# wwood/smafa

Hardware: AMD Instinct MI355X
Metric: query seqs/sec (DB residues/sec in `residues_per_s`) vs roofline, 10M x 60aa DB, d<=5 (higher is better)
Workload: dtype u32

## Files before the change

smafa_amd/csrc/engine.hip:

```cpp
#include <hipcub/hipcub.hpp>
#include <cmath>

#include <algorithm>
#include <atomic>
#include <cstdarg>
#include <cstdio>
#include <cstdlib>
#include <cstring>
#include <string>
#include <vector>

#include "engine.h"
#include "scan_plan.h"
#include "host/packed.h"
#include "kernels.hip.h"
#include "index.hip.h"
#include "join.hip.h"
#include "components.hip.h"
#include "levels.hip.h"
#include "density.hip.h"
#include "peaks.hip.h"
#include "neighbours.hip.h"

namespace smafa {
// ... 640 lines not shown
        x.probe_block[j] = j <= thr0 ? probe_block[j] : 0;
        x.probe_cols[j] = (uint32_t)ix.col_begin[x.probe_block[j]] | ((uint32_t)ix.col_begin[x.probe_block[j] + 1] << 16);
    }
    ScanArgs a{};
    a.n_subjects = (uint32_t)db->n;
    a.hits = d_rows;
    a.cap = rows_cap;
    a.count = d_count;
    a.order = db->d_order;
    int cur_dev = -1;
    if (hipGetDevice(&cur_dev) == hipSuccess) {
        db->launch_device = cur_dev;
        if (cur_dev != db->device) db->launches_off_device++;
    }
    const uint32_t *qrec = qs->qrec.as<uint32_t>();
    const uint32_t per_launch = (uint32_t)((1ull << 31) / kIndexGroup / x.n_probes);
    for (uint32_t qb = q_begin; qb < q_end;) {
        const uint32_t qe = q_end - qb > per_launch ? qb + per_launch : q_end;
        x.q_begin = qb;
        x.q_end = qe;
        const uint64_t groups = (uint64_t)(qe - qb) * x.n_probes;
        const uint64_t grid = (groups * kIndexGroup + kIndexWg - 1u) / kIndexWg;
        const bool launched = for_shape(db->shape(), [&](auto ps, auto pq, auto w) {
            constexpr int PS = decltype(ps)::value, PQ = decltype(pq)::value, W = decltype(w)::value;
            hipLaunchKernelGGL((index_probe_kernel<PS, PQ, W>), dim3((uint32_t)grid), dim3(kIndexWg), 0, db->stream, db->d_planes, qrec, x, a);
            note_kernel(db, "smafa::index_probe_kernel<%d, %d, %d>", PS, PQ, W);
            return true;
        });
        if (!launched) return set_error(SMAFA_ERR_INVALID, "no index probe for %u/%u planes x %u words", db->P, db->PQ, db->W);
        HIP_TRY(hipGetLastError());
        db->last_launches++;
        qb = qe;
    }
    db->plan_lazy = 0;
    db->plan_tiles = 0;
    db->plan_qblocks = 1;
    db->index_probes++;
    return SMAFA_OK;
}

static int launch_tiles(smafa_db *db, smafa_qset *qs, uint32_t q_begin, uint32_t q_end, uint32_t tile_begin,
                        uint32_t tile_end, uint32_t k_tight, uint32_t thr0, smafa_hit *d_rows, uint64_t rows_cap,
                        unsigned long long *publish, bool per_query_bounds = false, unsigned long long *own_counter = nullptr) {
    ScanArgs a;
    const uint32_t nq = q_end - q_begin, n_tiles = tile_end - tile_begin;
    const bool per_query = k_tight || per_query_bounds;
    const ScanPlan plan = plan_scan(db->shape(), db->knobs, {thr0, nq, d_rows == nullptr && k_tight == 1, d_rows != nullptr, per_query, {db->zone_hist}});
    const uint32_t T = plan.T;
    a.tile_begin = tile_begin;
    a.tile_end = tile_end;
    a.n_wg_tiles = (n_tiles + plan.wg_waves * T - 1) / (plan.wg_waves * T);
    a.n_subjects = (uint32_t)db->n;
    a.q_begin = q_begin;
    a.q_end = q_end;
    a.qb_size = query_block_size(db->qb_override, (uint32_t)db->n_cu, (n_tiles + kWgWaves * T - 1) / (kWgWaves * T), nq,
                                 plan.whole_chunks ? (uint32_t)kChunk : 1u);
    a.thr = per_query ? qs->thr.as<uint32_t>() : nullptr;
    a.thr0 = thr0;
    a.cnt = qs->cnt.as<uint32_t>();
    a.cnt_stride = db->L + 1;
    a.k_tight = k_tight;
    a.use_filter = db->knobs.use_filter ? 1u : 0u;
    a.hits = d_rows;
    a.cap = rows_cap;
    a.count = db->ctrs.as<unsigned long long>();
    a.done = publish ? reinterpret_cast<uint32_t *>(db->ctrs.as<uint8_t>() + 256) : nullptr;
    a.publish = publish;
    if (own_counter) {
        a.count = own_counter;
        a.done = nullptr;
        a.publish = nullptr;
    }
    a.order = db->d_order;
    a.zone = db->d_zone;
    a.zone_on = plan.zone_on ? 1u : 0u;
    {
        const uint32_t n1 = db->L > 32u ? std::min(db->L - 32u, 32u) : 0u, kb = (uint32_t)SMAFA_ZONE_KEY_BITS;
        const uint32_t xw = n1 >= 2u * kb ? kb : n1 / 2u;
        a.key_xmask = xw ? (uint32_t)((1ull << xw) - 1ull) : 0u;
        a.key_zlo = xw;
        a.key_gate = db->zone_key_gate >= 0                  ? (uint32_t)db->zone_key_gate
                     : db->alphabet == SMAFA_ALPHABET_AA ? (uint32_t)SMAFA_ZONE_KEY_GATE
                                                         : (uint32_t)SMAFA_ZONE_KEY_GATE_NT;
    }
    const uint64_t n_qblocks = (q_end - q_begin + a.qb_size - 1) / a.qb_size;
    const uint64_t range_bytes = (uint64_t)n_tiles * (plan.reported_lazy ? db->W : db->P * db->W) * 1024u;
    a.stream_once = (db->stream_nt && (n_qblocks == 1 || range_bytes >= (256ull << 20))) ? 1u : 0u;
    const uint64_t grid = n_qblocks * a.n_wg_tiles;
    if (grid > 0x7fffffffull)
        return set_error(SMAFA_ERR_INVALID, "scan grid too large (%llu workgroups)", (unsigned long long)grid);
    int cur_dev = -1;
    if (hipGetDevice(&cur_dev) == hipSuccess) {
        db->launch_device = cur_dev;
        if (cur_dev != db->device) db->launches_off_device++;
    }
    const std::string id = scan_kernel_name(plan, db->shape());
    note_kernel(db, "%s", id.c_str());
    if (plan.zone_on) note_kernel(db, "%s (zone level on)", id.c_str());
    if (!launch_scan(db, qs->qrec.as<uint32_t>(), a, (uint32_t)grid, plan)) return set_error(SMAFA_ERR_INVALID, "no kernel %s", id.c_str());
    db->plan_lazy = plan.reported_lazy ? 1u : 0u;
    db->plan_tiles = T;
    db->plan_qblocks = (uint32_t)n_qblocks;
    HIP_TRY(hipGetLastError());
    db->last_launches++;
    return SMAFA_OK;
}

static int scan_range(smafa_db *db, smafa_qset *qs, uint32_t q_begin, uint32_t q_end, uint32_t max_div,
                      uint32_t k_tight, smafa_hit *d_hits, uint64_t cap, unsigned long long *d_count, uint32_t tile_begin = 0) {
    const uint32_t nq = q_end - q_begin;
    db->last_launches = 0;
    db->timed = false;
    db->call_timed = false;
    if (nq == 0 || db->n == 0) {
        HIP_TRY(hipMemsetAsync(d_count, 0, sizeof(unsigned long long), db->stream));
        return SMAFA_OK;
    }
    int prc = maybe_resort(db);
    if (prc) return prc;
    unsigned long long *d_ctr = db->ctrs.as<unsigned long long>();
    const uint32_t thr0 = std::min<uint32_t>(max_div, db->L);
    const uint32_t n_tiles = (uint32_t)((db->n + kWaveTile - 1) / kWaveTile);
    if (k_tight == 0) {
        if (db->index_mode >= 2 && db->knobs.use_filter && nq > 64u && db->W <= (uint32_t)kIndexMaxWords && thr0 + 1u <= std::min<uint32_t>(kIndexMaxBlocks, db->L) &&
            db->n >= db->index_min_rows && db->n < (1ull << 31) && (!index_current(db) || db->index.B < thr0 + 1u)) {
            bool build = db->index_mode == 2;
            if (!build) {
                if (db->index_debt_generation != db->generation) db->index_debt_ms = 0.0, db->index_debt_generation = db->generation;
                db->index_debt_ms += (double)nq * (double)db->n * (double)(db->P * db->W) * 1.7e-12;
                build = db->index_debt_ms >= 0.3 + (double)(thr0 + 1u) * (double)db->n * 1.0e-7;
            }
            if (build && db->index_failed_generation != db->generation + 1u) {
                if (index_build(db, thr0 + 1u) != SMAFA_OK) {
                    log_line(1, "block index not built (%s): scanning as before", smafa_last_error());
                    index_drop(db);
                    db->index_failed_generation = db->generation + 1u;
                }
            }
        }
        uint8_t probe_block[kIndexMaxBlocks];
        if (index_plan(db, thr0, nq, probe_block)) {
            hipLaunchKernelGGL(fill_u32_kernel, dim3(1), dim3(64), 0, db->stream, (uint32_t *)d_count, 0u, (uint64_t)2);
            HIP_TRY(hipEventRecord(db->ev0, db->stream));
            int rc = index_probe(db, qs, q_begin, q_end, thr0, probe_block, d_hits, cap, d_count);
            if (rc) return rc;
            HIP_TRY(hipEventRecord(db->ev1, db->stream));
            db->timed = true;
            return SMAFA_OK;
        }
        const bool own = nq <= 64u;
        if (own) hipLaunchKernelGGL(fill_u32_kernel, dim3(1), dim3(64), 0, db->stream, (uint32_t *)d_count, 0u, (uint64_t)2);
        HIP_TRY(hipEventRecord(db->ev0, db->stream));
        int rc = launch_tiles(db, qs, q_begin, q_end, tile_begin, n_tiles, 0, thr0, d_hits, cap, own ? nullptr : d_count, false,
                              own ? d_count : nullptr);
        if (rc) return rc;
        HIP_TRY(hipEventRecord(db->ev1, db->stream));
        db->timed = true;
        return SMAFA_OK;
    }
    const bool count_first = k_tight >= db->count_first_k && !prefilter_prunes(db->shape(), db->knobs, thr0);
    const uint32_t sample_tiles = (count_first && db->kth_sample_div && n_tiles >= db->kth_sample_min_tiles &&
                                   n_tiles / db->kth_sample_div >= 1u &&
                                   (uint64_t)k_tight * 4u <= (uint64_t)(n_tiles / db->kth_sample_div) * kWaveTile)
                                      ? n_tiles / db->kth_sample_div : 0u;
    uint64_t scratch_rows = 0;
    if (!count_first || sample_tiles) {
// ... 1480 lines not shown
```

smafa_amd/csrc/kernels.hip.h:

```cpp
#pragma once

#include <type_traits>
#include <hip/hip_runtime.h>
#include <stdint.h>

#include "../../include/smafa_amd.h"
#include "scan_plan.h"

namespace smafa {

constexpr int kStageRows = 256;
__host__ __device__ constexpr int scan_min_waves(int ps, int w, int t) {
    const int regs = t * ps * w * 4 + 40;
    return regs <= 64 ? 8 : regs <= 80 ? 6 : regs <= 96 ? 5 : regs <= 128 ? 4 : regs <= 168 ? 3 : 2;
}
#ifndef SMAFA_CASCADE
#define SMAFA_CASCADE 1
#endif
#ifndef SMAFA_WIDE_AND_PAIR
#define SMAFA_WIDE_AND_PAIR 1
#endif
#ifndef SMAFA_SIGN_COMPARE
#define SMAFA_SIGN_COMPARE 1
#endif
// ... 680 lines not shown
                    }
                }
            }
        }
        if (more) commit(buf ^ 1, qc + kChunk);
        __syncthreads();
        if (!SEED && a.hits) flush_rows(a, rs, buf);
    }
    if (!SEED) finish_rows(a);
}

__device__ __forceinline__ void emit_direct(const ScanArgs &a, uint32_t q, uint32_t pos, uint32_t dist) {
    smafa_hit h;
    h.query = q;
    h.subject = a.order[pos];
    h.dist = dist;
    const unsigned long long together = __ballot(1);
    const int first = __builtin_ctzll(together);
    unsigned long long g = 0;
    if ((int)__lane_id() == first) g = atomicAdd(a.count, (unsigned long long)__builtin_popcountll(together));
    g = shfl_u64(g, first) + lanes_below(together);
    if (g < a.cap) a.hits[g] = h;
}

constexpr int kZoneTiles = SMAFA_ZONE_TILES;

#ifndef SMAFA_ZONE_WAVES_10
#define SMAFA_ZONE_WAVES_10 5
#endif
#ifndef SMAFA_ZONE_SGPR_ZONE
#define SMAFA_ZONE_SGPR_ZONE 1
#endif
#ifndef SMAFA_ZONE_VGPR_MASK
#define SMAFA_ZONE_VGPR_MASK 6
#endif
#ifndef SMAFA_ZONE_OPAQUE_BUF
#define SMAFA_ZONE_OPAQUE_BUF 1
#endif
#ifndef SMAFA_ZONE_FULL_DMA
#define SMAFA_ZONE_FULL_DMA 1
#endif
#ifndef SMAFA_ZONE_NLIVE
#define SMAFA_ZONE_NLIVE 1
#endif
#ifndef SMAFA_ZONE_WAVES_4
#define SMAFA_ZONE_WAVES_4 6
#endif
#ifndef SMAFA_ZONE_WAVES_6
#define SMAFA_ZONE_WAVES_6 6
#endif
#ifndef SMAFA_ZONE_WAVES_DIRECT_AA
#define SMAFA_ZONE_WAVES_DIRECT_AA 7
#endif
#ifndef SMAFA_ZONE_KEYS
#define SMAFA_ZONE_KEYS 3
#endif
#ifndef SMAFA_ZONE_KEY_BITS
#define SMAFA_ZONE_KEY_BITS 12
#endif
#ifndef SMAFA_ZONE_KEY_GATE
#define SMAFA_ZONE_KEY_GATE 3
#endif
#ifndef SMAFA_ZONE_KEY_GATE_NT
#define SMAFA_ZONE_KEY_GATE_NT 2
#endif
#ifndef SMAFA_ZONE_KEY_HOIST
#define SMAFA_ZONE_KEY_HOIST 1
#endif
#ifndef SMAFA_ZONE_L2_LANES
#define SMAFA_ZONE_L2_LANES 1
#endif
#ifndef SMAFA_ZONE_F1_HOME_AA
#define SMAFA_ZONE_F1_HOME_AA 1
#endif
#ifndef SMAFA_ZONE_F1_HOME_NT
#define SMAFA_ZONE_F1_HOME_NT 0
#endif
__host__ __device__ constexpr int zone_f1_home(int ps, int w, bool direct) {
    return !(SMAFA_ZONE_L2_LANES && direct && w == 2 && SMAFA_ZONE_KEYS > 0) ? 0 : ps == 5 ? SMAFA_ZONE_F1_HOME_AA : SMAFA_ZONE_F1_HOME_NT;
}
#ifndef SMAFA_ZONE_KEY_BATCH
#define SMAFA_ZONE_KEY_BATCH 1
#endif
__host__ __device__ constexpr int zone_key_sets(int w, bool direct) { return direct && w == 2 ? SMAFA_ZONE_KEYS : 0; }
static_assert(SMAFA_ZONE_KEYS == 0 || SMAFA_ZONE_KEYS == 2 || SMAFA_ZONE_KEYS == 3, "SMAFA_ZONE_KEYS: 0, 2 or 3");
static_assert(SMAFA_ZONE_KEY_BITS >= 8 && SMAFA_ZONE_KEY_BITS <= 16, "SMAFA_ZONE_KEY_BITS: 8..16");

__host__ __device__ constexpr int zone_min_waves(int ps, int w, bool direct = false) {
    return (direct && ps == 5 && w == 2 && SMAFA_ZONE_TILES == 4) ? SMAFA_ZONE_WAVES_DIRECT_AA
           : ps * w <= 4 ? SMAFA_ZONE_WAVES_4 : (ps == 3 && w == 2) ? SMAFA_ZONE_WAVES_6 : ps * w <= 10 ? SMAFA_ZONE_WAVES_10 : 4;
}

template <int PS, int PQ, int W, bool FIXED, bool DIRECT = false>
__global__ __launch_bounds__(kZoneWgWaves * 64, zone_min_waves(PS, W, DIRECT)) void scan_zone_kernel(const uint4 *__restrict__ planes,
                                                           const uint32_t *__restrict__ qrec, ScanArgs a) {
    static_assert(FIXED || !DIRECT, "per-query bounds keep the staged form");
    constexpr int T = zone_tiles(PS, W, DIRECT);
    constexpr int RS = qrec_stride(PQ, W);
    constexpr int RV = RS / 4;
    constexpr int WGW = kZoneWgWaves;
    constexpr int NT = WGW * 64;
    constexpr int NV = (kChunk * RV + NT - 1) / NT;
    constexpr int FP = filter_plane(PQ);
    constexpr int BS = bound_slot(W);
    constexpr bool kPair = SMAFA_AND_PAIR && W > 1;
    __shared__ uint4 stage[2][kChunk * RV];
    __shared__ uint32_t nu_lds[2][kChunk];
    __shared__ RowStageT<(WGW == 1 ? 64 : kStageRows)> rs;
    constexpr int NS = zone_key_sets(W, DIRECT);
    constexpr int KB = SMAFA_ZONE_KEY_BITS;
    constexpr int KW = (1 << KB) / 32;
    __shared__ uint4 keymap[NS ? WGW * T * NS * KW / 4 : 1];
    constexpr int kF1Home = NS > 0 ? zone_f1_home(PS, W, DIRECT) : 0;
    constexpr bool kL2Lanes = NS > 0 && W == 2 && SMAFA_ZONE_L2_LANES;
    __shared__ uint4 f1_lds[kF1Home == 1 ? WGW * T * 64 : 1];
    int buf = 0;

    const uint32_t tid = threadIdx.x;
    const uint32_t lane = tid & 63u;
    const uint32_t wave = tid >> 6;
    if ((!DIRECT || NS == 0) && tid == 0) rs.n[0] = rs.n[1] = 0;
    const uint32_t wg_tile = blockIdx.x % a.n_wg_tiles;
    const uint32_t qblock = blockIdx.x / a.n_wg_tiles;
    const uint32_t tile0 = (uint32_t)__builtin_amdgcn_readfirstlane((int)(a.tile_begin + (wg_tile * WGW + wave) * T));
    const bool active = tile0 < a.tile_end;
    const uint32_t n_live = active ? min((uint32_t)T, a.tile_end - tile0) : 0u;
    const uint32_t q0 = a.q_begin + qblock * a.qb_size;
    const uint32_t q1 = min(q0 + a.qb_size, a.q_end);

    uint4 f0[T];
    uint4 f1_reg[kF1Home == 2 ? T : 1];
    auto load_filter = [&]() {
#pragma unroll
        for (int t = 0; t < T; t++) {
            const bool live = SMAFA_ZONE_NLIVE ? (uint32_t)t < n_live : tile0 + t < a.tile_end;
            f0[t] = planes[(size_t)(live ? tile0 + t : a.tile_begin) * (PS * W * 64) + (FP * W) * 64 + lane];
            if constexpr (kF1Home == 2) f1_reg[t] = planes[(size_t)(live ? tile0 + t : a.tile_begin) * (PS * W * 64) + (FP * W + 1) * 64 + lane];
        }
    };
    load_filter();
    uint4 vz = make_uint4(0u, 0u, 0u, 0u);
    if (lane < (uint32_t)T && tile0 + lane < a.tile_end) vz = a.zone[tile0 + lane];
    uint32_t zc0[T], zm0[T];
#pragma unroll
    for (int t = 0; t < T; t++) {
        zc0[t] = (uint32_t)__builtin_amdgcn_readlane((int)vz.x, t);
        zm0[t] = (uint32_t)__builtin_amdgcn_readlane((int)vz.y, t);
    }
    constexpr bool kMaskInVgpr = PS * W <= SMAFA_ZONE_VGPR_MASK;
    uint32_t zmv[T];
#pragma unroll
    for (int t = 0; t < T; t++) {
        zmv[t] = zm0[t];
        if (kMaskInVgpr) asm volatile("v_mov_b32 %0, %1" : "=v"(zmv[t]) : "s"(zm0[t]));
    }
    const bool zone_w1 = W > 1 && __ballot(vz.w != 0u) != 0ull;
    uint32_t zc1s[T], zm1s[T];
#pragma unroll
    for (int t = 0; t < T; t++) {
        zc1s[t] = NS > 0 ? (uint32_t)__builtin_amdgcn_readlane((int)vz.z, t) : 0u;
        zm1s[t] = NS > 0 ? (uint32_t)__builtin_amdgcn_readlane((int)vz.w, t) : 0u;
    }

    auto key_y = [&](uint32_t w0) -> uint32_t { return w0 >> (32 - KB); };
    auto key_x = [&](uint32_t w1) -> uint32_t { return w1 & a.key_xmask; };
    auto key_z = [&](uint32_t w1) -> uint32_t { return __builtin_amdgcn_ubfe(w1, a.key_zlo, KB); };
    constexpr bool kHoist = NS > 0 && SMAFA_ZONE_KEY_HOIST;
    bool key_hoist = false;
    if constexpr (kHoist) {
        uint32_t shared_keys = 0;
#pragma unroll
        for (int t = 0; t < T; t++) shared_keys |= key_y(zm0[t]) | key_x(zm1s[t]) | (NS > 2 ? key_z(zm1s[t]) : 0u);
        key_hoist = shared_keys == 0u;
    }
    uint32_t *const km = reinterpret_cast<uint32_t *>(keymap) + (size_t)__builtin_amdgcn_readfirstlane((int)wave) * (T * NS * KW);
    uint4 *const f1_home = f1_lds + (kF1Home == 1 ? (size_t)__builtin_amdgcn_readfirstlane((int)wave) * (T * 64) : 0);
    if constexpr (NS > 0) {
        uint4 *const km4 = reinterpret_cast<uint4 *>(km);
#pragma unroll
        for (int i = 0; i < T * NS * KW / 4; i += 64)
            if (i + 64 <= T * NS * KW / 4 || i + (int)lane < T * NS * KW / 4) km4[i + lane] = make_uint4(0u, 0u, 0u, 0u);
        __builtin_amdgcn_wave_barrier();
        asm volatile("s_waitcnt lgkmcnt(0)" ::: "memory");
#pragma unroll
        for (int t = 0; t < T; t++) {
            const bool live = (uint32_t)t < n_live;
            uint4 f1;
            if constexpr (kF1Home == 2) f1 = f1_reg[t];
            else f1 = planes[(size_t)(live ? tile0 + t : a.tile_begin) * (PS * W * 64) + (FP * W + 1) * 64 + lane];
            if constexpr (kF1Home == 1) f1_home[t * 64 + lane] = f1;
            const uint32_t w0[4] = {f0[t].x, f0[t].y, f0[t].z, f0[t].w};
            const uint32_t w1[4] = {f1.x, f1.y, f1.z, f1.w};
#pragma unroll
            for (int k = 0; k < 4; k++) {
                const uint32_t ky = key_y(w0[k]), kx = key_x(w1[k]);
                atomicOr(&km[(t * NS + 0) * KW + (ky >> 5)], 1u << (ky & 31u));
                atomicOr(&km[(t * NS + 1) * KW + (kx >> 5)], 1u << (kx & 31u));
                if (NS > 2) {
                    const uint32_t kz = key_z(w1[k]);
                    atomicOr(&km[(t * NS + (NS > 2 ? 2 : 0)) * KW + (kz >> 5)], 1u << (kz & 31u));
                }
            }
        }
        __builtin_amdgcn_wave_barrier();
        asm volatile("s_waitcnt lgkmcnt(0)" ::: "memory");
    }

    auto dma = [&](int b, uint32_t qc) {
        const uint32_t nqc = SMAFA_ZONE_FULL_DMA ? (uint32_t)kChunk : min((uint32_t)kChunk, q1 - qc);
        const uint4 *src = reinterpret_cast<const uint4 *>(qrec + (size_t)qc * RS);
#pragma unroll
        for (int v = 0; v < NV; v++) {
            const uint32_t idx = tid + v * NT;
            if (idx < nqc * RV)
                __builtin_amdgcn_global_load_lds((const __attribute__((address_space(1))) void *)(src + idx),
                                                 (__attribute__((address_space(3))) void *)(&stage[b][wave * 64 + v * NT]), 16, 0, 0);
        }
    };
    const uint32_t nu0 = ~a.thr0;
    auto load_bound = [&](uint32_t qc) -> uint32_t {
        return tid < min((uint32_t)kChunk, q1 - qc) ? ~ld_relaxed(a.thr + qc + tid) : 0u;
    };
    uint32_t nu_next = 0;
    auto read_record = [&](const uint4 *rec, uint32_t(&qw)[RS]) {
#pragma unroll
        for (int v = 0; v < RV; v++) {
            const uint4 x = rec[v];
            qw[4 * v + 0] = x.x;
            qw[4 * v + 1] = x.y;
            qw[4 * v + 2] = x.z;
            qw[4 * v + 3] = x.w;
        }
    };
    auto stream_compare = [&](uint32_t tile, const uint32_t(&qw)[RS], uint32_t q, int parity) {
        const uint32_t U = ~qw[BS];
        const uint4 *src = planes + (size_t)tile * (PS * W * 64) + lane;
        uint32_t d[4] = {0u, 0u, 0u, 0u};
#pragma unroll
        for (int w = 0; w < W; w++) {
            uint32_t extra = 0;
#pragma unroll
            for (int p = PS; p < PQ; p++) extra |= qw[qslot(PQ, W, p, w)];
            uint32_t m0 = extra, m1 = extra, m2 = extra, m3 = extra;
#pragma unroll
            for (int p = 0; p < PS; p++) {
                const uint4 v = src[(p * W + w) * 64];
                const uint32_t qv = qw[qslot(PQ, W, p, w)];
                m0 = or_xor(m0, v.x, qv);
                m1 = or_xor(m1, v.y, qv);
                m2 = or_xor(m2, v.z, qv);
                m3 = or_xor(m3, v.w, qv);
            }
            d[0] += __builtin_popcount(m0);
            d[1] += __builtin_popcount(m1);
            d[2] += __builtin_popcount(m2);
            d[3] += __builtin_popcount(m3);
        }
        const uint32_t subj0 = tile * kWaveTile + lane * 4u;
#pragma unroll
        for (int k = 0; k < 4; k++)
            if (d[k] <= U && subj0 + k < a.n_subjects) {
                if (DIRECT) emit_direct(a, q, subj0 + k, d[k]);
                else emit(a, rs, parity, q, subj0 + k, d[k]);
            }
    };
    auto load_head = [&](uint32_t qc) -> uint2 {
        return *reinterpret_cast<const uint2 *>(qrec + (size_t)(qc + lane) * RS);
    };
    uint2 head_next = make_uint2(0u, 0u);

    if (!DIRECT) {
        if (q0 < q1) {
            dma(0, q0);
            if (!FIXED && tid < (uint32_t)kChunk) nu_lds[0][tid] = load_bound(q0);
        }
        asm volatile("s_waitcnt vmcnt(0)" ::: "memory");
        __syncthreads();
    } else if (q0 < q1) {
        head_next = load_head(q0);
    }
    bool filter_on = a.use_filter != 0;
    uint32_t chunk_no = 0;
    for (uint32_t qc = q0; qc < q1; qc += kChunk, buf ^= 1, chunk_no++) {
        const uint32_t nqc = min((uint32_t)kChunk, q1 - qc);
        const bool more = qc + kChunk < q1;
        const uint2 head_cur = head_next;
        if (more) {
            if (DIRECT) {
                head_next = load_head(qc + kChunk);
            } else {
                dma(buf ^ 1, qc + kChunk);
                if (!FIXED) nu_next = load_bound(qc + kChunk);
            }
        }
        if (active) {
            const bool probe = a.use_filter && (filter_on || (chunk_no & 15u) == 0);
            if (probe) {
                uint32_t passes = 0;
                uint4 head = make_uint4(0u, 0u, 0u, 0u);
                if (DIRECT) head.x = head_cur.x, head.y = head_cur.y;
                else if (lane < nqc) head = stage[buf][lane * RV];
                const uint32_t hq0 = head.x, hq1 = W > 1 ? head.y : 0u;
                const uint32_t hnu = lane < nqc ? (FIXED ? nu0 : nu_lds[buf][lane]) : 0u;
                uint32_t nl = n_live;
                asm volatile("" : "+s"(nl));
                if (!SMAFA_ZONE_SGPR_ZONE) asm volatile("" : "+v"(vz.x), "+v"(vz.y));
                auto zone_keys = [&](auto slot) -> unsigned long long {
                    constexpr uint32_t t = decltype(slot)::value;
                    const uint32_t zc = SMAFA_ZONE_SGPR_ZONE ? zc0[t] : (uint32_t)__builtin_amdgcn_readlane((int)vz.x, (int)t);
                    const uint32_t zm = SMAFA_ZONE_SGPR_ZONE ? zm0[t] : (uint32_t)__builtin_amdgcn_readlane((int)vz.y, (int)t);
                    const uint32_t d0 = (hq0 ^ zc) & (kMaskInVgpr ? zmv[t] : zm);
                    uint32_t u = __builtin_popcount(d0) + hnu;
                    uint32_t d1 = 0;
                    if (zone_w1) {
                        const uint32_t zc1 = NS > 0 ? zc1s[t] : (uint32_t)__builtin_amdgcn_readlane((int)vz.z, (int)t);
                        const uint32_t zm1 = NS > 0 ? zm1s[t] : (uint32_t)__builtin_amdgcn_readlane((int)vz.w, (int)t);
                        d1 = (hq1 ^ zc1) & zm1;
                        u += __builtin_popcount(d1);
                    }
                    unsigned long long m = __ballot((int32_t)u < 0);
                    if constexpr (NS > 0) {
                        if ((uint32_t)__builtin_popcountll(m) >= a.key_gate) {
                            bool pass = false;
                            if ((int32_t)u < 0) {
                                const uint32_t s0 = hq0 ^ d0, s1 = hq1 ^ d1;
                                const uint32_t ky = key_y(s0), kx = key_x(s1);
                                const uint32_t vy = km[(t * NS + 0) * KW + (ky >> 5)];
                                const uint32_t vx = km[(t * NS + 1) * KW + (kx >> 5)];
                                uint32_t found = ((vy >> (ky & 31u)) & 1u) + ((vx >> (kx & 31u)) & 1u);
                                if (NS > 2) {
                                    const uint32_t kz = key_z(s1);
                                    const uint32_t vz_ = km[(t * NS + (NS > 2 ? 2 : 0)) * KW + (kz >> 5)];
                                    found += (vz_ >> (kz & 31u)) & 1u;
                                }
                                pass = found + ~u >= (uint32_t)NS;
                            }
                            m = __ballot(pass);
                        }
                    }
                    return m;
                };
                auto survivors = [&](auto slot, unsigned long long m) {
                    constexpr uint32_t t = decltype(slot)::value;
                    const uint32_t tile = tile0 + t;
                    const uint4 ft = f0[t];
                    while (m != 0ull) {
                        const int i = __builtin_ctzll(m);
                        asm("s_bitset0_b64 %0, %1" : "+s"(m) : "s"(i));
                        const uint32_t q0w = (uint32_t)__builtin_amdgcn_readlane((int)hq0, i);
                        const uint32_t nu = FIXED ? nu0 : (uint32_t)__builtin_amdgcn_readlane((int)hnu, i);
                        const uint32_t u0 = __builtin_popcount(ft.x ^ q0w) + nu;
                        const uint32_t u1 = __builtin_popcount(ft.y ^ q0w) + nu;
                        const uint32_t u2 = __builtin_popcount(ft.z ^ q0w) + nu;
                        const uint32_t u3 = __builtin_popcount(ft.w ^ q0w) + nu;
                        if (__ballot((int32_t)(or3(u0, u1, u2) | u3) < 0) == 0ull) continue;
                        uint32_t tile_r = tile;
                        asm volatile("" : "+s"(tile_r));
#if SMAFA_ZONE_OPAQUE_BUF
                        int buf_r = __builtin_amdgcn_readfirstlane(buf);
                        asm volatile("" : "+s"(buf_r));
#define SMAFA_ZONE_BUF buf_r
#else
#define SMAFA_ZONE_BUF buf
#endif
                        uint32_t qw[RS];
                        if constexpr (kL2Lanes) {
                            const uint32_t q1w = (uint32_t)__builtin_amdgcn_readlane((int)hq1, i);
                            uint4 v;
                            if constexpr (kF1Home == 1) v = f1_home[t * 64 + lane];
                            else if constexpr (kF1Home == 2) v = f1_reg[t];
                            else v = planes[(size_t)tile_r * (PS * W * 64) + (FP * W + 1) * 64 + lane];
                            const uint32_t m0 = or_xor(ft.x ^ q0w, v.x, q1w), m1 = or_xor(ft.y ^ q0w, v.y, q1w);
                            const uint32_t m2 = or_xor(ft.z ^ q0w, v.z, q1w), m3 = or_xor(ft.w ^ q0w, v.w, q1w);
                            if (kPair) {
                                const uint32_t sign = (__builtin_popcount(m0 & m1) + nu) | (__builtin_popcount(m2 & m3) + nu);
                                if (__ballot((int32_t)sign < 0) == 0ull) continue;
                            }
                            const uint32_t each = or3(__builtin_popcount(m0) + nu, __builtin_popcount(m1) + nu,
                                                      __builtin_popcount(m2) + nu) |
                                                  (__builtin_popcount(m3) + nu);
                            if (__ballot((int32_t)each < 0) == 0ull) continue;
                            read_record(reinterpret_cast<const uint4 *>(qrec + (size_t)(qc + (uint32_t)i) * RS), qw);
                            qw[BS] = nu;
                            passes++;
                            stream_compare(tile_r, qw, qc + (uint32_t)i, SMAFA_ZONE_BUF);
                            continue;
                        }
                        if (DIRECT) read_record(reinterpret_cast<const uint4 *>(qrec + (size_t)(qc + (uint32_t)i) * RS), qw);
                        else read_record(&stage[SMAFA_ZONE_BUF][(uint32_t)i * RV], qw);
                        qw[BS] = nu;
                        uint32_t m0 = ft.x ^ qw[0], m1 = ft.y ^ qw[0], m2 = ft.z ^ qw[0], m3 = ft.w ^ qw[0];
                        if (W > 1) {
                            const uint4 *src = planes + (size_t)tile_r * (PS * W * 64) + (FP * W) * 64 + lane;
#pragma unroll
                            for (int w = 1; w < W; w++) {
                                const uint4 v = src[w * 64];
                                m0 = or_xor(m0, v.x, qw[qslot(PQ, W, FP, w)]);
                                m1 = or_xor(m1, v.y, qw[qslot(PQ, W, FP, w)]);
                                m2 = or_xor(m2, v.z, qw[qslot(PQ, W, FP, w)]);
                                m3 = or_xor(m3, v.w, qw[qslot(PQ, W, FP, w)]);
                            }
                            if (kPair) {
                                const uint32_t sign = (__builtin_popcount(m0 & m1) + nu) | (__builtin_popcount(m2 & m3) + nu);
                                if (__ballot((int32_t)sign < 0) == 0ull) continue;
                            }
                            const uint32_t each = or3(__builtin_popcount(m0) + nu, __builtin_popcount(m1) + nu,
                                                      __builtin_popcount(m2) + nu) |
                                                  (__builtin_popcount(m3) + nu);
                            if (__ballot((int32_t)each < 0) == 0ull) continue;
                        }
                        passes++;
                        stream_compare(tile_r, qw, qc + (uint32_t)i, SMAFA_ZONE_BUF);
#undef SMAFA_ZONE_BUF
                    }
                };
                static_assert(T <= 8, "tile slots are spelled out below");
                auto each_slot = [&](auto &&f) {
                    f(std::integral_constant<uint32_t, 0>{});
                    if constexpr (T > 1) f(std::integral_constant<uint32_t, 1>{});
                    if constexpr (T > 2) f(std::integral_constant<uint32_t, 2>{});
                    if constexpr (T > 3) f(std::integral_constant<uint32_t, 3>{});
                    if constexpr (T > 4) f(std::integral_constant<uint32_t, 4>{});
                    if constexpr (T > 5) f(std::integral_constant<uint32_t, 5>{});
                    if constexpr (T > 6) f(std::integral_constant<uint32_t, 6>{});
                    if constexpr (T > 7) f(std::integral_constant<uint32_t, 7>{});
                };
                static_assert(!kHoist || (SMAFA_ZONE_NLIVE && SMAFA_ZONE_SGPR_ZONE),
                              "the two-phase form of the key-test kernels is written for SMAFA_ZONE_NLIVE = SMAFA_ZONE_SGPR_ZONE = 1");
                if constexpr (kHoist) {
                    unsigned long long ms[T];
                    if (key_hoist) {
                        const uint32_t ky = key_y(hq0), kx = key_x(hq1), kz = NS > 2 ? key_z(hq1) : 0u;
                        typedef const __attribute__((address_space(3))) uint32_t *lds_u32;
                        const uint32_t km_lds = (uint32_t)(uintptr_t)(__attribute__((address_space(3))) void *)km;
                        auto word_of = [&](uint32_t key) -> uint32_t {
                            uint32_t at;
                            asm("v_lshl_add_u32 %0, %1, 2, %2" : "=v"(at) : "v"(key >> 5), "s"(km_lds));
                            return at;
                        };
                        const uint32_t ay = word_of(ky), ax = word_of(kx), az = NS > 2 ? word_of(kz) : 0u;
                        const unsigned long long in_block = ~0ull >> (64u - nqc);
                        auto hoisted = [&](auto with_w1) {
                            if constexpr (SMAFA_ZONE_KEY_BATCH) {
                                uint32_t u[T];
                                bool test = false;
                                each_slot([&](auto slot) {
                                    constexpr uint32_t t = decltype(slot)::value;
                                    u[t] = __builtin_popcount((hq0 ^ zc0[t]) & (kMaskInVgpr ? zmv[t] : zm0[t])) + nu0;
                                    if (decltype(with_w1)::value) u[t] += __builtin_popcount((hq1 ^ zc1s[t]) & zm1s[t]);
                                    const unsigned long long m = __builtin_amdgcn_ballot_w64((int32_t)u[t] < 0) & in_block;
                                    ms[t] = t == 0u || nl > t ? m : 0ull;
                                    test = test || (uint32_t)__builtin_popcountll(ms[t]) >= a.key_gate;
                                });
                                if (test) {
                                    uint32_t g[T][3];
                                    each_slot([&](auto slot) {
                                        constexpr uint32_t t = decltype(slot)::value;
                                        g[t][0] = g[t][1] = g[t][2] = 0u;
                                        if ((int32_t)u[t] < 0) {
                                            g[t][0] = *(lds_u32)(uintptr_t)(ay + ((t * NS + 0) * KW) * 4u);
                                            g[t][1] = *(lds_u32)(uintptr_t)(ax + ((t * NS + 1) * KW) * 4u);
                                            if (NS > 2) g[t][2] = *(lds_u32)(uintptr_t)(az + ((t * NS + (NS > 2 ? 2 : 0)) * KW) * 4u);
                                        }
                                    });
                                    each_slot([&](auto slot) {
                                        constexpr uint32_t t = decltype(slot)::value;
                                        uint32_t found = __builtin_amdgcn_ubfe(g[t][0], ky, 1) + __builtin_amdgcn_ubfe(g[t][1], kx, 1);
                                        if (NS > 2) found += __builtin_amdgcn_ubfe(g[t][2], kz, 1);
                                        ms[t] &= __builtin_amdgcn_ballot_w64((int32_t)(u[t] - found) < -(int32_t)NS);
                                    });
                                }
                            } else {
                            auto one = [&](auto slot) -> unsigned long long {
                                constexpr uint32_t t = decltype(slot)::value;
                                uint32_t u = __builtin_popcount((hq0 ^ zc0[t]) & (kMaskInVgpr ? zmv[t] : zm0[t])) + nu0;
                                if (decltype(with_w1)::value) u += __builtin_popcount((hq1 ^ zc1s[t]) & zm1s[t]);
                                unsigned long long m = __builtin_amdgcn_ballot_w64((int32_t)u < 0) & in_block;
                                if ((uint32_t)__builtin_popcountll(m) >= a.key_gate) {
                                    if ((int32_t)u < 0) {
                                        uint32_t found = __builtin_amdgcn_ubfe(*(lds_u32)(uintptr_t)(ay + ((t * NS + 0) * KW) * 4u), ky, 1) +
                                                         __builtin_amdgcn_ubfe(*(lds_u32)(uintptr_t)(ax + ((t * NS + 1) * KW) * 4u), kx, 1);
                                        if (NS > 2) found += __builtin_amdgcn_ubfe(*(lds_u32)(uintptr_t)(az + ((t * NS + (NS > 2 ? 2 : 0)) * KW) * 4u), kz, 1);
                                        u -= found;
                                    }
                                    asm("" : "+v"(u));
                                    m &= __builtin_amdgcn_ballot_w64((int32_t)u < -(int32_t)NS);
                                }
                                return m;
                            };
                            each_slot([&](auto slot) {
                                constexpr uint32_t t = decltype(slot)::value;
                                ms[t] = t == 0u || nl > t ? one(slot) : 0ull;
                            });
                            }
                        };
                        if (zone_w1) hoisted(std::true_type{});
                        else hoisted(std::false_type{});
                    } else {
                        each_slot([&](auto slot) {
                            constexpr uint32_t t = decltype(slot)::value;
                            ms[t] = t == 0u || nl > t ? zone_keys(slot) : 0ull;
                        });
                    }
                    each_slot([&](auto slot) { survivors(slot, ms[decltype(slot)::value]); });
                } else {
                    each_slot([&](auto slot) {
                        constexpr uint32_t t = decltype(slot)::value;
                        if (SMAFA_ZONE_NLIVE ? nl > t : tile0 + t < a.tile_end) survivors(slot, zone_keys(slot));
                    });
                }
                filter_on = passes * 5u <= nqc * 8u;
            } else {
                for (uint32_t t = 0; t < (uint32_t)T; t++) {
                    const uint32_t tile = tile0 + t;
                    if (SMAFA_ZONE_NLIVE ? t >= n_live : tile >= a.tile_end) break;
                    uint4 s[PS * W];
                    uint32_t tile_d = tile;
                    asm volatile("" : "+s"(tile_d));
                    const uint4 *src = planes + (size_t)(SMAFA_ZONE_NLIVE ? tile_d : tile) * (PS * W * 64) + lane;
#pragma unroll
                    for (int i = 0; i < PS * W; i++) s[i] = src[i * 64];
                    const uint4 *rec = DIRECT ? reinterpret_cast<const uint4 *>(qrec + (size_t)qc * RS) : &stage[buf][0];
                    for (uint32_t i = 0; i < nqc; i++, rec += RV) {
                        uint32_t qw[RS];
                        read_record(rec, qw);
                        const uint32_t U = FIXED ? a.thr0 : ~nu_lds[buf][i];
                        uint32_t d[4];
#pragma unroll
                        for (int w = 0; w < W; w++) {
                            uint32_t extra = 0;
#pragma unroll
                            for (int p = PS; p < PQ; p++) extra |= qw[qslot(PQ, W, p, w)];
                            uint32_t m0 = extra, m1 = extra, m2 = extra, m3 = extra;
#pragma unroll
                            for (int p = 0; p < PS; p++) {
                                const uint4 v = s[p * W + w];
                                const uint32_t qv = qw[qslot(PQ, W, p, w)];
                                m0 = or_xor(m0, v.x, qv);
                                m1 = or_xor(m1, v.y, qv);
                                m2 = or_xor(m2, v.z, qv);
                                m3 = or_xor(m3, v.w, qv);
                            }
                            d[0] = (w ? d[0] : 0u) + __builtin_popcount(m0);
                            d[1] = (w ? d[1] : 0u) + __builtin_popcount(m1);
                            d[2] = (w ? d[2] : 0u) + __builtin_popcount(m2);
                            d[3] = (w ? d[3] : 0u) + __builtin_popcount(m3);
                        }
                        const uint32_t subj0 = tile * kWaveTile + lane * 4u;
#pragma unroll
                        for (int k = 0; k < 4; k++)
                            if (d[k] <= U && subj0 + k < a.n_subjects) {
                                if (DIRECT) emit_direct(a, qc + i, subj0 + k, d[k]);
                                else emit(a, rs, buf, qc + i, subj0 + k, d[k]);
                            }
                    }
                }
                load_filter();
            }
        }
        if (!DIRECT) {
            if (more && !FIXED && tid < (uint32_t)kChunk) nu_lds[buf ^ 1][tid] = nu_next;
            asm volatile("s_waitcnt vmcnt(0)" ::: "memory");
            __syncthreads();
            if (a.hits) flush_rows(a, rs, buf);
        }
    }
    finish_rows(a);
}

template <int PS, int PQ, int W>
__global__ __launch_bounds__(256) void scan_zone_few_kernel(const uint4 *__restrict__ planes,
                                                            const uint32_t *__restrict__ qrec, ScanArgs a) {
    constexpr int T = kFewTiles;
    constexpr int RS = qrec_stride(PQ, W);
    constexpr int RV = RS / 4;
    constexpr int FP = filter_plane(PQ);
    constexpr int BS = bound_slot(W);
    constexpr bool kPair = SMAFA_AND_PAIR && W > 1;
    __shared__ RowStage rs;
    const uint32_t tid = threadIdx.x;
// ... 932 lines not shown
```

smafa_amd/csrc/scan_plan.h:

```cpp
#pragma once

#include <cstdint>
#include <cstdio>
#include <string>

namespace smafa {

constexpr int kWaveTile = 256;
constexpr int kWgWaves = 4;
constexpr int kChunk = 64;
#ifndef SMAFA_SUM_FOLD
#define SMAFA_SUM_FOLD 1
#endif

constexpr int round_up4(int x) { return (x + 3) & ~3; }
constexpr int qrec_stride(int planes, int words) { return round_up4(planes * words + 1); }

#ifndef SMAFA_ZONE_TILES
#define SMAFA_ZONE_TILES 4
#endif
#ifndef SMAFA_ZONE_TILES_DIRECT_AA
#define SMAFA_ZONE_TILES_DIRECT_AA 2
#endif
constexpr int zone_tiles(int ps, int w, bool direct) {
    return SMAFA_ZONE_TILES != 4 ? SMAFA_ZONE_TILES : (direct && ps == 5 && w == 2 ? SMAFA_ZONE_TILES_DIRECT_AA : 4);
}
#ifndef SMAFA_ZONE_WG_WAVES
#define SMAFA_ZONE_WG_WAVES 2
#endif
constexpr int kZoneWgWaves = SMAFA_ZONE_WG_WAVES;
#ifndef SMAFA_FEW_TILES
#define SMAFA_FEW_TILES 4
#endif
constexpr int kFewTiles = SMAFA_FEW_TILES;

constexpr int kWideTiles = 4;
constexpr int kWideStage = 768;
constexpr bool wide_fits(int planes, int words) { return qrec_stride(planes, words) / 4 <= kWideStage; }
constexpr int kGenericTiles = 4;

struct ScanKnobs {
    bool lazy = true;
    bool use_filter = true;
    bool wide_one = true;
    uint32_t wide_from = 5;
    uint32_t tiles_override = 0;
    int zone = 1;
    double zone_loose = 0.3;
    bool zone_direct = true;
    double prune_p = 2e-3;
    bool lazy_fold = true;
    bool fold3 = true;
};

struct ScanShape {
    uint32_t P, PQ, W, L;
};

inline double binom_tail(uint32_t bits, uint32_t bound) {
    if (bound >= bits) return 1.0;
    double term = 1.0, tail = 0.0;
    for (uint32_t i = 0; i <= bound; i++) {
        tail += term;
        term = term * (double)(bits - i) / (double)(i + 1);
    }
    for (uint32_t i = 0; i < bits; i++) tail *= 0.5;
    return tail;
}

inline bool prefilter_prunes(const ScanShape &s, const ScanKnobs &k, uint32_t bound) {
    const uint32_t cols = s.L < 32u ? s.L : 32u;
    return bound < cols && binom_tail(cols, bound) <= k.prune_p;
}

inline bool fold_rejects(const ScanShape &s, const ScanKnobs &k, uint32_t bound) {
    if (!k.lazy_fold || s.W != 2 || s.L < 56) return false;
    const uint32_t second = s.L - 32u;
    const uint32_t unrelated = (3u * second + 2u * (32u - second)) / 4u;
    return bound * 2u <= unrelated + 1u || bound <= 14u;
}

inline double zone_pass_share(const uint64_t *hist, uint32_t thr0) {
    double tiles = 0.0, pass = 0.0;
    for (uint32_t b = 0; b <= 64; b++) {
        if (!hist[b]) continue;
        tiles += (double)hist[b];
        pass += (double)hist[b] * binom_tail(b, thr0);
    }
    return tiles > 0.0 ? pass / tiles : 1.0;
}

struct ZoneShare {
    const uint64_t *hist = nullptr;
    double value = 1.0;
    double at(uint32_t thr0) const { return hist ? zone_pass_share(hist, thr0) : value; }
};

inline bool zone_pays(const ScanShape &s, const ScanKnobs &k, uint32_t thr0, bool prunes, const ZoneShare &share) {
    if (!k.lazy || !k.use_filter) return false;
    if (k.zone != 1) return k.zone == 2;
    const double pays = s.W <= 4 && s.P * s.W >= 20 ? 0.4 : 0.6;
    return share.at(thr0) < (prunes ? pays : k.zone_loose);
}

struct ScanLaunch {
    uint32_t thr0;
    uint32_t nq;
    bool seed;
    bool has_rows;
// ... 86 lines not shown
```

Before: 24.42 million.

## Add launch-time key gate, early head load, undef key loads, interleaved key layout

```diff
diff --git a/smafa_amd/csrc/engine.hip b/smafa_amd/csrc/engine.hip
--- a/smafa_amd/csrc/engine.hip
+++ b/smafa_amd/csrc/engine.hip
@@ -746,6 +746,8 @@
         a.key_gate = db->zone_key_gate >= 0                  ? (uint32_t)db->zone_key_gate
                      : db->alphabet == SMAFA_ALPHABET_AA ? (uint32_t)SMAFA_ZONE_KEY_GATE
                                                          : (uint32_t)SMAFA_ZONE_KEY_GATE_NT;
+        if (plan.family == ScanFamily::zone && plan.direct && db->W == 2)
+            a.key_gate = launch_key_gate(a.key_gate, db->zone_key_gate >= 0, zone_pass_share(db->zone_hist, thr0));
     }
     const uint64_t n_qblocks = (q_end - q_begin + a.qb_size - 1) / a.qb_size;
     const uint64_t range_bytes = (uint64_t)n_tiles * (plan.reported_lazy ? db->W : db->P * db->W) * 1024u;
diff --git a/smafa_amd/csrc/kernels.hip.h b/smafa_amd/csrc/kernels.hip.h
--- a/smafa_amd/csrc/kernels.hip.h
+++ b/smafa_amd/csrc/kernels.hip.h
@@ -786,6 +786,12 @@
 #ifndef SMAFA_ZONE_KEY_BATCH
 #define SMAFA_ZONE_KEY_BATCH 1
 #endif
+#ifndef SMAFA_ZONE_KEY_UNDEF
+#define SMAFA_ZONE_KEY_UNDEF 1
+#endif
+#ifndef SMAFA_ZONE_HEAD_EARLY
+#define SMAFA_ZONE_HEAD_EARLY 1
+#endif
 __host__ __device__ constexpr int zone_key_sets(int w, bool direct) { return direct && w == 2 ? SMAFA_ZONE_KEYS : 0; }
 static_assert(SMAFA_ZONE_KEYS == 0 || SMAFA_ZONE_KEYS == 2 || SMAFA_ZONE_KEYS == 3, "SMAFA_ZONE_KEYS: 0, 2 or 3");
 static_assert(SMAFA_ZONE_KEY_BITS >= 8 && SMAFA_ZONE_KEY_BITS <= 16, "SMAFA_ZONE_KEY_BITS: 8..16");
@@ -845,6 +851,13 @@
     load_filter();
     uint4 vz = make_uint4(0u, 0u, 0u, 0u);
     if (lane < (uint32_t)T && tile0 + lane < a.tile_end) vz = a.zone[tile0 + lane];
+    auto load_head = [&](uint32_t qc) -> uint2 {
+        return *reinterpret_cast<const uint2 *>(qrec + (size_t)(qc + lane) * RS);
+    };
+    uint2 head_next = make_uint2(0u, 0u);
+    constexpr bool kHeadEarly = DIRECT && zone_key_sets(W, DIRECT) > 0 && SMAFA_ZONE_HEAD_EARLY;
+    if constexpr (kHeadEarly)
+        if (q0 < q1) head_next = load_head(q0);
     uint32_t zc0[T], zm0[T];
 #pragma unroll
     for (int t = 0; t < T; t++) {
@@ -877,6 +890,14 @@
         for (int t = 0; t < T; t++) shared_keys |= key_y(zm0[t]) | key_x(zm1s[t]) | (NS > 2 ? key_z(zm1s[t]) : 0u);
         key_hoist = shared_keys == 0u;
     }
+    constexpr bool kIlv = NS > 0 && zone_key_interleaved(T);
+    constexpr int LT = kIlv ? zone_key_log2(T) : 0;
+    auto kword = [](uint32_t k, uint32_t t, uint32_t s) -> uint32_t { return zone_key_word(k, t, s, T, NS, KW); };
+    auto kbit = [](uint32_t k, uint32_t t) -> uint32_t { return zone_key_bit(k, t, T); };
+    auto unset = [](uint32_t &g) {
+        if constexpr (SMAFA_ZONE_KEY_UNDEF) asm volatile("" : "=v"(g));
+        else g = 0u;
+    };
     uint32_t *const km = reinterpret_cast<uint32_t *>(keymap) + (size_t)__builtin_amdgcn_readfirstlane((int)wave) * (T * NS * KW);
     uint4 *const f1_home = f1_lds + (kF1Home == 1 ? (size_t)__builtin_amdgcn_readfirstlane((int)wave) * (T * 64) : 0);
     if constexpr (NS > 0) {
@@ -898,11 +919,11 @@
 #pragma unroll
             for (int k = 0; k < 4; k++) {
                 const uint32_t ky = key_y(w0[k]), kx = key_x(w1[k]);
-                atomicOr(&km[(t * NS + 0) * KW + (ky >> 5)], 1u << (ky & 31u));
-                atomicOr(&km[(t * NS + 1) * KW + (kx >> 5)], 1u << (kx & 31u));
+                atomicOr(&km[kword(ky, t, 0)], 1u << kbit(ky, t));
+                atomicOr(&km[kword(kx, t, 1)], 1u << kbit(kx, t));
                 if (NS > 2) {
                     const uint32_t kz = key_z(w1[k]);
-                    atomicOr(&km[(t * NS + (NS > 2 ? 2 : 0)) * KW + (kz >> 5)], 1u << (kz & 31u));
+                    atomicOr(&km[kword(kz, t, NS > 2 ? 2 : 0)], 1u << kbit(kz, t));
                 }
             }
         }
@@ -968,11 +989,6 @@
                 else emit(a, rs, parity, q, subj0 + k, d[k]);
             }
     };
-    auto load_head = [&](uint32_t qc) -> uint2 {
-        return *reinterpret_cast<const uint2 *>(qrec + (size_t)(qc + lane) * RS);
-    };
-    uint2 head_next = make_uint2(0u, 0u);
-
     if (!DIRECT) {
         if (q0 < q1) {
             dma(0, q0);
@@ -980,10 +996,11 @@
         }
         asm volatile("s_waitcnt vmcnt(0)" ::: "memory");
         __syncthreads();
-    } else if (q0 < q1) {
+    } else if (!kHeadEarly && q0 < q1) {
         head_next = load_head(q0);
     }
     bool filter_on = a.use_filter != 0;
+    const uint32_t key_form = (uint32_t)__builtin_amdgcn_readfirstlane(zone_w1 ? 1 : NS > 0 && a.key_gate == 0u ? 2 : 0);
     uint32_t chunk_no = 0;
     for (uint32_t qc = q0; qc < q1; qc += kChunk, buf ^= 1, chunk_no++) {
         const uint32_t nqc = min((uint32_t)kChunk, q1 - qc);
@@ -1029,13 +1046,13 @@
                             if ((int32_t)u < 0) {
                                 const uint32_t s0 = hq0 ^ d0, s1 = hq1 ^ d1;
                                 const uint32_t ky = key_y(s0), kx = key_x(s1);
-                                const uint32_t vy = km[(t * NS + 0) * KW + (ky >> 5)];
-                                const uint32_t vx = km[(t * NS + 1) * KW + (kx >> 5)];
-                                uint32_t found = ((vy >> (ky & 31u)) & 1u) + ((vx >> (kx & 31u)) & 1u);
+                                const uint32_t vy = km[kword(ky, t, 0)];
+                                const uint32_t vx = km[kword(kx, t, 1)];
+                                uint32_t found = ((vy >> kbit(ky, t)) & 1u) + ((vx >> kbit(kx, t)) & 1u);
                                 if (NS > 2) {
                                     const uint32_t kz = key_z(s1);
-                                    const uint32_t vz_ = km[(t * NS + (NS > 2 ? 2 : 0)) * KW + (kz >> 5)];
-                                    found += (vz_ >> (kz & 31u)) & 1u;
+                                    const uint32_t vz_ = km[kword(kz, t, NS > 2 ? 2 : 0)];
+                                    found += (vz_ >> kbit(kz, t)) & 1u;
                                 }
                                 pass = found + ~u >= (uint32_t)NS;
                             }
@@ -1139,28 +1156,47 @@
                         const uint32_t km_lds = (uint32_t)(uintptr_t)(__attribute__((address_space(3))) void *)km;
                         auto word_of = [&](uint32_t key) -> uint32_t {
                             uint32_t at;
-                            asm("v_lshl_add_u32 %0, %1, 2, %2" : "=v"(at) : "v"(key >> 5), "s"(km_lds));
+                            asm("v_lshl_add_u32 %0, %1, 2, %2" : "=v"(at) : "v"(key >> (5 - LT)), "s"(km_lds));
                             return at;
                         };
                         const uint32_t ay = word_of(ky), ax = word_of(kx), az = NS > 2 ? word_of(kz) : 0u;
                         const unsigned long long in_block = ~0ull >> (64u - nqc);
-                        auto hoisted = [&](auto with_w1) {
+                        auto hoisted = [&](auto with_w1, auto always) {
                             if constexpr (SMAFA_ZONE_KEY_BATCH) {
                                 uint32_t u[T];
-                                bool test = false;
+                                bool test = decltype(always)::value;
                                 each_slot([&](auto slot) {
                                     constexpr uint32_t t = decltype(slot)::value;
                                     u[t] = __builtin_popcount((hq0 ^ zc0[t]) & (kMaskInVgpr ? zmv[t] : zm0[t])) + nu0;
                                     if (decltype(with_w1)::value) u[t] += __builtin_popcount((hq1 ^ zc1s[t]) & zm1s[t]);
                                     const unsigned long long m = __builtin_amdgcn_ballot_w64((int32_t)u[t] < 0) & in_block;
                                     ms[t] = t == 0u || nl > t ? m : 0ull;
-                                    test = test || (uint32_t)__builtin_popcountll(ms[t]) >= a.key_gate;
+                                    if constexpr (!decltype(always)::value) test = test || (uint32_t)__builtin_popcountll(ms[t]) >= a.key_gate;
                                 });
-                                if (test) {
+                                if constexpr (kIlv) {
+                                    if (test) {
+                                        uint32_t any = u[0];
+                                        each_slot([&](auto slot) { any |= u[decltype(slot)::value]; });
+                                        uint32_t g[3];
+                                        unset(g[0]), unset(g[1]), unset(g[2]);
+                                        if ((int32_t)any < 0) {
+                                            g[0] = *(lds_u32)(uintptr_t)(ay + (0 * T * KW) * 4u);
+                                            g[1] = *(lds_u32)(uintptr_t)(ax + (1 * T * KW) * 4u);
+                                            if (NS > 2) g[2] = *(lds_u32)(uintptr_t)(az + ((NS > 2 ? 2 : 0) * T * KW) * 4u);
+                                        }
+                                        uint32_t found_all = __builtin_amdgcn_ubfe(g[0], ky << LT, T) | (__builtin_amdgcn_ubfe(g[1], kx << LT, T) << 8);
+                                        if (NS > 2) found_all |= __builtin_amdgcn_ubfe(g[2], kz << LT, T) << 16;
+                                        each_slot([&](auto slot) {
+                                            constexpr uint32_t t = decltype(slot)::value;
+                                            const uint32_t found = __builtin_popcount(found_all & (0x010101u << t));
+                                            ms[t] &= __builtin_amdgcn_ballot_w64((int32_t)(u[t] - found) < -(int32_t)NS);
+                                        });
+                                    }
+                                } else if (test) {
                                     uint32_t g[T][3];
                                     each_slot([&](auto slot) {
                                         constexpr uint32_t t = decltype(slot)::value;
-                                        g[t][0] = g[t][1] = g[t][2] = 0u;
+                                        unset(g[t][0]), unset(g[t][1]), unset(g[t][2]);
                                         if ((int32_t)u[t] < 0) {
                                             g[t][0] = *(lds_u32)(uintptr_t)(ay + ((t * NS + 0) * KW) * 4u);
                                             g[t][1] = *(lds_u32)(uintptr_t)(ax + ((t * NS + 1) * KW) * 4u);
@@ -1175,6 +1211,7 @@
                                     });
                                 }
                             } else {
+                            (void)always;
                             auto one = [&](auto slot) -> unsigned long long {
                                 constexpr uint32_t t = decltype(slot)::value;
                                 uint32_t u = __builtin_popcount((hq0 ^ zc0[t]) & (kMaskInVgpr ? zmv[t] : zm0[t])) + nu0;
@@ -1182,9 +1219,11 @@
                                 unsigned long long m = __builtin_amdgcn_ballot_w64((int32_t)u < 0) & in_block;
                                 if ((uint32_t)__builtin_popcountll(m) >= a.key_gate) {
                                     if ((int32_t)u < 0) {
-                                        uint32_t found = __builtin_amdgcn_ubfe(*(lds_u32)(uintptr_t)(ay + ((t * NS + 0) * KW) * 4u), ky, 1) +
-                                                         __builtin_amdgcn_ubfe(*(lds_u32)(uintptr_t)(ax + ((t * NS + 1) * KW) * 4u), kx, 1);
-                                        if (NS > 2) found += __builtin_amdgcn_ubfe(*(lds_u32)(uintptr_t)(az + ((t * NS + (NS > 2 ? 2 : 0)) * KW) * 4u), kz, 1);
+                                        constexpr auto off = [](uint32_t set) { return (kIlv ? set * T * KW : (t * NS + set) * KW) * 4u; };
+                                        auto bit = [](uint32_t key) { return kIlv ? (key << LT) + t : key; };
+                                        uint32_t found = __builtin_amdgcn_ubfe(*(lds_u32)(uintptr_t)(ay + off(0)), bit(ky), 1) +
+                                                         __builtin_amdgcn_ubfe(*(lds_u32)(uintptr_t)(ax + off(1)), bit(kx), 1);
+                                        if (NS > 2) found += __builtin_amdgcn_ubfe(*(lds_u32)(uintptr_t)(az + off(NS > 2 ? 2 : 0)), bit(kz), 1);
                                         u -= found;
                                     }
                                     asm("" : "+v"(u));
@@ -1198,8 +1237,9 @@
                             });
                             }
                         };
-                        if (zone_w1) hoisted(std::true_type{});
-                        else hoisted(std::false_type{});
+                        if (key_form == 2u) hoisted(std::false_type{}, std::true_type{});
+                        else if (key_form == 1u) hoisted(std::true_type{}, std::false_type{});
+                        else hoisted(std::false_type{}, std::false_type{});
                     } else {
                         each_slot([&](auto slot) {
                             constexpr uint32_t t = decltype(slot)::value;
diff --git a/smafa_amd/csrc/scan_plan.h b/smafa_amd/csrc/scan_plan.h
--- a/smafa_amd/csrc/scan_plan.h
+++ b/smafa_amd/csrc/scan_plan.h
@@ -25,6 +25,25 @@
 constexpr int zone_tiles(int ps, int w, bool direct) {
     return SMAFA_ZONE_TILES != 4 ? SMAFA_ZONE_TILES : (direct && ps == 5 && w == 2 ? SMAFA_ZONE_TILES_DIRECT_AA : 4);
 }
+#ifndef SMAFA_ZONE_KEY_INTERLEAVE
+#define SMAFA_ZONE_KEY_INTERLEAVE 0
+#endif
+constexpr bool zone_key_interleaved(int T) { return SMAFA_ZONE_KEY_INTERLEAVE && T > 1 && T <= 8 && (T & (T - 1)) == 0; }
+constexpr int zone_key_log2(int T) { return T <= 1 ? 0 : 1 + zone_key_log2(T / 2); }
+constexpr uint32_t zone_key_word(uint32_t k, uint32_t t, uint32_t s, int T, int NS, int KW) {
+    return zone_key_interleaved(T) ? s * (uint32_t)(T * KW) + (k >> (5 - zone_key_log2(T))) : (t * (uint32_t)NS + s) * (uint32_t)KW + (k >> 5);
+}
+constexpr uint32_t zone_key_bit(uint32_t k, uint32_t t, int T) {
+    return zone_key_interleaved(T) ? (k & (32u / (uint32_t)T - 1u)) * (uint32_t)T + t : k & 31u;
+}
+#ifndef SMAFA_ZONE_KEY_GATE_LAUNCH
+#define SMAFA_ZONE_KEY_GATE_LAUNCH 1
+#endif
+inline uint32_t launch_key_gate(uint32_t gate, bool set_at_run_time, double share) {
+    if (!SMAFA_ZONE_KEY_GATE_LAUNCH || set_at_run_time || gate > 64u) return gate;
+    return share * 64.0 >= 2.0 * (double)gate ? 0u : gate;
+}
+
 #ifndef SMAFA_ZONE_WG_WAVES
 #define SMAFA_ZONE_WG_WAVES 2
 #endif
```

Result: no change. 24.24 million (-0.7%).
